# gwlucastrig/gridfour

Hardware: NVIDIA B200
Metric: GVRS tile decode GB/s of raw samples (config 3 shard, 180x240 tiles) (higher is better)
Workload: dtype int32

## Files before the change

### gridfour_b200/csrc/g4_lsop_fast.cu

```cuda
#include <cuda.h>
#include <cstdio>
#include <type_traits>
#include "g4_kernels.h"
#include "g4_predict.cuh"
#include "g4_lsop_common.cuh"

namespace g4 {

namespace {

constexpr int kTextThreads = 512;
constexpr int kTextThreadsSmall = 256;
constexpr uint32_t kTextSmallTile = 16384;
constexpr uint32_t kTextSubBits = 320;
constexpr int kExcWords = 128;
constexpr int kExcCap = (kExcWords - 2) / 2;
constexpr uint32_t kTextLookback = 96;
constexpr int kStageWordsPerThread = 22;
constexpr int kSpillWords = 8;
constexpr int kResidGuard = 256;
constexpr float kMagicHalf = 6291456.0f;
constexpr float kMagicHalfUp = 6291456.5f;
constexpr float kMagicInt = 12582912.0f;
constexpr float kRange = 2097152.0f;

__device__ __forceinline__ uint32_t smem_u32(const void* p) { return uint32_t(__cvta_generic_to_shared(p)); }
__host__ __device__ constexpr size_t text_fast_bytes(uint32_t stageWords) {
  return (offsetof(CanonFastShared, sw) + size_t(stageWords + 8u) * 4u + 127u) & ~size_t(127);
}
__device__ __forceinline__ void mbar_init(uint32_t bar, uint32_t count) {
  asm volatile("mbarrier.init.shared::cta.b64 [%0], %1;" ::"r"(bar), "r"(count));
}
__device__ __forceinline__ void mbar_expect_tx(uint32_t bar, uint32_t bytes) {
  asm volatile("mbarrier.arrive.expect_tx.shared::cta.b64 _, [%0], %1;" ::"r"(bar), "r"(bytes) : "memory");
}
__device__ __forceinline__ void mbar_wait(uint32_t bar, uint32_t parity) {
  uint32_t done = 0;
  while (!done)
    asm volatile("{ .reg .pred p; mbarrier.try_wait.parity.shared::cta.b64 p, [%1], %2; selp.u32 %0, 1, 0, p; }"
                 : "=r"(done)
                 : "r"(bar), "r"(parity)
                 : "memory");
}

__device__ __forceinline__ uint32_t image_offset(uint32_t w, int logW, uint32_t P, uint32_t k) {
  const uint32_t rr = k / w, pp = k - rr * w;
  return (rr + (pp >> logW)) * P + pp;
}

__device__ inline uint32_t warp_scan_inplace(int32_t* p, int n, uint32_t carry, int stride = 1) {
  const int lane = threadIdx.x & 31;
  for (int i0 = 0; i0 < n; i0 += 32) {
    const int i = i0 + lane;
    const uint32_t x = i < n ? uint32_t(p[i * stride]) : 0u;
    const uint32_t inc = warp_inclusive_scan(x);
    if (i < n) p[i * stride] = int32_t(carry + inc);
    carry += __shfl_sync(0xffffffffu, inc, 31);
  }
  __syncwarp();
  return carry;
}

__global__ void __launch_bounds__(kThreads, 3) lsop2_head_kernel(LsopFastArgs A, uint32_t maxPackBytes, int listBegin, int listEnd) {
  extern __shared__ __align__(16) unsigned char headSmem[];
  const DecodeArgs& a = A.a;
  const int lane = threadIdx.x & 31, warp = threadIdx.x >> 5;
  const int R = A.g.R, C = A.g.C;
  const uint32_t nInit = uint32_t(4 * R + 2 * C - 9);
  const size_t perWarp = ((sizeof(CanonWarpShared) + 15) & ~size_t(15)) + ((size_t(nInit) * 4 + 15) & ~size_t(15));
  CanonWarpShared& W = *reinterpret_cast<CanonWarpShared*>(headSmem + perWarp * warp);
  int32_t* init = reinterpret_cast<int32_t*>(headSmem + perWarp * warp + ((sizeof(CanonWarpShared) + 15) & ~size_t(15)));
  const int li = listBegin + blockIdx.x * kWarps + warp;
  if (li >= listEnd || li >= *a.listCount) return;
  const int tIdx = a.list[li];
  uint8_t* m = A.meta + size_t(tIdx) * kLsopMetaBytes;
  if (lane == 0) {
    *reinterpret_cast<uint32_t*>(m) = 0;
    A.exc[size_t(tIdx) * kExcWords] = 0;
  }
  const TileView t = tile_view(a.band, a.grid, tIdx);
  const uint8_t* packing = a.arena + a.offsets[tIdx];
  const uint32_t len = a.lens[tIdx];
  LsHeaderInfo h = parse_ls_header(packing, len, A.coef + size_t(tIdx) * 12, lane == 0);
  if (lane == 0 && a.lsopCks && h.ok && h.hasChecksum) { a.lsopCks[2 * tIdx] = 1u; a.lsopCks[2 * tIdx + 1] = h.valueChecksum; }
  if (!h.ok) {
    if (lane == 0) a.status[tIdx] = G4_ERR_FORMAT;
    return;
  }
  if (h.type != 2 || len + 96u > maxPackBytes) {
    if (lane == 0) A.defer[atomicAdd(A.deferCount, 1)] = tIdx;
    return;
  }
  BitSrc src;
  src.init(packing, len);
  canon_warp_parse_header(W, src, h.headerSize * 8u);
  int status = W.error ? G4_ERR_FORMAT : G4_OK;
  uint32_t endBit = 0;
  if (status == G4_OK) {
    uint32_t eb = 0, nv = 0;
    auto emit = [&](uint32_t k, int32_t v) { init[k] = v; };
    const bool ok = canon_warp_decode_text(W, src, W.textStart, nInit, emit, &eb, &nv) && nv == nInit;
    __syncwarp();
    if (lane == 0) {
      if (!ok) W.error = 1;
      W.textStart = eb;
    }
    __syncwarp();
    if (W.error) status = G4_ERR_FORMAT;
    endBit = W.textStart;
  }
  if (status == G4_OK) {
    canon_warp_parse_header(W, src, endBit);
    if (W.error) status = G4_ERR_FORMAT;
    else {
      for (int i = lane; i < kCanonSymbols; i += 32) {
        m[8 + i] = W.lens[i];
        reinterpret_cast<uint16_t*>(m + kLsopMetaSorted)[i] = W.sorted[i];
      }
      if (lane < 17) {
        reinterpret_cast<uint16_t*>(m + kLsopMetaFirst)[lane] = W.firstCode[lane];
        reinterpret_cast<uint16_t*>(m + kLsopMetaCount)[lane] = W.count[lane];
        reinterpret_cast<uint16_t*>(m + kLsopMetaOffset)[lane] = W.offset[lane];
      }
      if (lane == 0) *reinterpret_cast<uint32_t*>(m) = W.textStart;
    }
  }
  if (status == G4_OK) {
    int32_t* sA = init;
    int32_t* sB = sA + (C - 1);
    int32_t* sC = sB + (R - 1);
    int32_t* sD = sC + (C - 1);
    int32_t* sE = sD + (R - 2);
    const uint32_t seed = uint32_t(h.seed);
    warp_scan_inplace(sA, C - 1, seed);
    warp_scan_inplace(sB, R - 1, seed);
    warp_scan_inplace(sC, C - 1, uint32_t(sB[0]) - seed);
    for (int i = lane; i < C - 1; i += 32) sC[i] = int32_t(uint32_t(sC[i]) + uint32_t(sA[i]));
    __syncwarp();
    warp_scan_inplace(sD, R - 2, uint32_t(sC[0]) - uint32_t(sB[0]));
    warp_scan_inplace(sE, R - 2, uint32_t(sC[C - 3]) - uint32_t(sC[C - 4]), 2);
    warp_scan_inplace(sE + 1, R - 2, uint32_t(sC[C - 2]) - uint32_t(sC[C - 3]), 2);
    int32_t* row0 = t.row(0);
    int32_t* row1 = t.row(1);
    for (int c = lane; c < C; c += 32) {
      row0[c] = c ? sA[c - 1] : int32_t(seed);
      row1[c] = c ? sC[c - 1] : sB[0];
    }
    int4* side = A.side + size_t(tIdx) * R;
    for (int r = lane; r < R; r += 32) {
      int4 s;
      if (r == 0) s = make_int4(int32_t(seed), sA[0], 0, 0);
      else if (r == 1) s = make_int4(sB[0], sC[0], 0, 0);
      else s = make_int4(sB[r - 1], int32_t(uint32_t(sB[r - 1]) + uint32_t(sD[r - 2])), sE[2 * (r - 2)], sE[2 * (r - 2) + 1]);
      side[r] = s;
    }
  }
  if (lane == 0) a.status[tIdx] = status;
}

struct ByteTileSink {
  static constexpr bool kPacked = true;
  uint8_t* tile;
  uint32_t* exc;
  int w;
  int logW;
  uint32_t P, Wm1;
  uint32_t addr;
  uint32_t rowBase;
  int left;
  int kAddr;
  int head;
  int cnt;
  uint64_t q;
  int excK, excSlot;
  int32_t excV;

  __device__ __forceinline__ void init(uint8_t* img, uint32_t* e, const LsopFastGeom& geom) {
    tile = img;
    exc = e;
    logW = geom.logW;
    w = geom.C - 4;
    P = uint32_t(geom.P);
    Wm1 = uint32_t(geom.W - 1);
  }
  __device__ __forceinline__ void begin(uint32_t k0) {
    const int rr = int(k0) / w, pp = int(k0) - rr * w;
    rowBase = uint32_t(rr) * P;
    const uint32_t a0 = rowBase + (uint32_t(pp) >> logW) * P + uint32_t(pp);
    head = pp & 3;
    addr = a0 & ~3u;
    left = w - (pp & ~3);
    kAddr = int(k0) - head;
    cnt = head;
    q = 0;
    excK = -1;
    excSlot = 0;
    excV = 0;
  }
  __device__ __forceinline__ int cur_k() const { return kAddr + cnt; }
  __device__ __forceinline__ void store_word() {
    if (head) {
      for (int i = head; i < 4; i++) tile[addr + i] = uint8_t(q >> (8 * i));
      head = 0;
    } else *reinterpret_cast<uint32_t*>(tile + addr) = uint32_t(q);
    q >>= 32;
    cnt -= 4;
    kAddr += 4;
    step();
  }
  __device__ __forceinline__ void step() {
    addr += 4;
    left -= 4;
    if ((addr & Wm1) == 0u) {
      addr += P;
      if (left == 0) {
        rowBase += P;
        addr = rowBase;
        left = w;
      }
    } else if (__builtin_expect(left == 0, 0)) {
      rowBase += P;
      addr = rowBase;
      left = w;
    }
  }
  __device__ __forceinline__ void put_word(uint32_t dw, int lo, int hi) {
    if (lo == 0 && hi >= 4) *reinterpret_cast<uint32_t*>(tile + addr) = dw;
    else
      for (int b = lo; b < hi && b < 4; b++) tile[addr + b] = uint8_t(dw >> (8 * b));
    step();
  }
  __device__ __forceinline__ void push(uint32_t bytes, int n) {
    q |= uint64_t(bytes) << (8 * cnt);
    cnt += n;
    if (cnt >= 4) store_word();
  }
  __device__ __forceinline__ int add_exception(int k, int32_t v) {
    const uint32_t slot = atomicAdd(exc, 1u);
    if (slot < uint32_t(kExcCap)) {
      exc[2 + 2 * slot] = uint32_t(k);
      exc[3 + 2 * slot] = uint32_t(v);
    }
    excK = k;
    excV = v;
    excSlot = int(slot);
    return int(slot);
  }
  __device__ __forceinline__ void put_rare(int32_t v) {
    add_exception(cur_k(), v);
    push(0u, 1);
  }
  __device__ __forceinline__ void amend(int nb, uint32_t bits) {
    const int kp = cur_k() - 1;
    if (kp == excK) {
      excV = int32_t((uint32_t(excV) << nb) | bits);
      if (excSlot < kExcCap) exc[3 + 2 * excSlot] = uint32_t(excV);
      return;
    }
    uint32_t b;
    if (cnt > head) {
      const int sh = 8 * (cnt - 1);
      b = uint32_t(q >> sh) & 0xffu;
      q &= ~(0xffull << sh);
    } else {
      const uint32_t o = image_offset(uint32_t(w), logW, P, uint32_t(kp));
      b = tile[o];
      tile[o] = 0;
    }
    add_exception(kp, int32_t(((b - 128u) << nb) | bits));
  }
  __device__ __forceinline__ void end() {
    for (int i = head; i < cnt; i++) tile[addr + i] = uint8_t(q >> (8 * i));
  }
};

constexpr int kSubRare = 4;
constexpr int kSubOverflow = 8;

struct PosCursor {
  uint32_t lo, hi, next, pos;
  __device__ __forceinline__ void init(const uint32_t* sw, uint32_t p) {
    const uint32_t i = p >> 5;
    lo = sw[i];
    hi = sw[i + 1];
    next = i + 2;
    pos = p;
  }
  __device__ __forceinline__ uint32_t peek() const { return __funnelshift_r(lo, hi, pos); }
  __device__ __forceinline__ void skip(const uint32_t* sw, uint32_t n) {
    const uint32_t np = pos + n;
    if ((np ^ pos) & 32u) {
      lo = hi;
      hi = sw[next++];
    }
    pos = np;
  }
};

struct ByteAcc {
  uint32_t acc, qc8, w;
  __device__ __forceinline__ void init() { acc = 0; qc8 = 0; w = 0; }
  __device__ __forceinline__ void append(uint32_t m24, uint32_t n8, uint32_t* slot, uint32_t slotWords, uint32_t* spill) {
    const uint32_t out = __funnelshift_l(acc, m24, qc8);
    acc = __funnelshift_r(acc, m24, n8);
    qc8 += n8;
    if (qc8 >= 32u) {
      if (w < slotWords) slot[w] = out;
      else if (w - slotWords < uint32_t(kSpillWords)) spill[w - slotWords] = out;
      w++;
      qc8 -= 32u;
    }
  }
  __device__ __forceinline__ void finish(uint32_t* slot, uint32_t slotWords, uint32_t* spill) {
    if (qc8) {
      const uint32_t out = acc >> (32u - qc8);
      if (w < slotWords) slot[w] = out;
      else if (w - slotWords < uint32_t(kSpillWords)) spill[w - slotWords] = out;
      w++;
    }
  }
};

__device__ __forceinline__ void text_stage_sub(const CanonFastShared& S, uint32_t nBits, uint32_t start, uint32_t limit, uint32_t* slot,
                                               uint32_t slotWords, uint32_t* spill, uint32_t* endOut, uint32_t* cntOut, int* flagOut) {
  PosCursor cur;
  cur.init(S.sw, start);
  const int lastFull = int(limit) - kFastLutBits;
  uint32_t c = 0, end;
  int flag = 0;
  ByteAcc A;
  A.init();
  for (;;) {
    if (int(cur.pos) <= lastFull) {
      const uint32_t m = S.mlut[cur.peek() & ((1u << kFastLutBits) - 1u)];
      const uint32_t n = m >> 28;
      if (n) {
        cur.skip(S.sw, (m >> 24) & 15u);
        c += n;
        A.append(m & 0xffffffu, (m >> 25) & 0x18u, slot, slotWords, spill);
        continue;
      }
    }
    const uint32_t e = S.lut[cur.peek() & ((1u << kFastLutBits) - 1u)];
    uint32_t byte;
    if (e - 1u < 0x7fffu) {
      if (cur.pos >= limit) { end = cur.pos; break; }
      cur.skip(S.sw, e >> 9);
      byte = e & 0xffu;
    } else {
      const uint32_t p0 = cur.pos;
      uint32_t after;
      const int sym = canon_fast_rare_symbol(S, e, p0, nBits, &after);
      if (sym < 0) { flag = 2; end = p0; break; }
      if (sym == kSymEsc2 || sym == kSymEsc8) {
        after += sym == kSymEsc2 ? 2u : 8u;
        if (after > nBits) { flag = 2; end = p0; break; }
        flag |= kSubRare;
        cur.init(S.sw, after);
        continue;
      }
      if (p0 >= limit) { end = p0; break; }
      if (sym == kSymEot) { flag |= 1; end = after; break; }
      if (sym == kSymNull) { flag |= kSubRare; byte = 0u; }
      else byte = uint32_t(sym);
      cur.init(S.sw, after);
    }
    c++;
    A.append(byte, 8u, slot, slotWords, spill);
  }
  A.finish(slot, slotWords, spill);
  if (A.w > slotWords + uint32_t(kSpillWords)) flag |= kSubOverflow;
  *endOut = end;
  *cntOut = c;
  *flagOut = flag;
}

__device__ __forceinline__ bool text_write_sub(const CanonFastShared& S, uint32_t nBits, uint32_t start, uint32_t limit, uint32_t k0,
                                            ByteTileSink& sink) {
  BitCursor cur;
  cur.init(S, start, limit);
  sink.begin(k0);
  bool have = false, ok = true;
  for (;;) {
    if (cur.rem >= kFastLutBits) {
      const uint32_t m = S.mlut[cur.peek() & ((1u << kFastLutBits) - 1u)];
      const uint32_t n = m >> 28;
      if (n) {
        cur.skip(S, (m >> 24) & 15u);
        sink.push(m & 0xffffffu, int(n));
        have = true;
        continue;
      }
    }
    const uint32_t e = S.lut[cur.peek() & ((1u << kFastLutBits) - 1u)];
    if (e - 1u < 0x7fffu) {
      if (cur.rem <= 0) break;
      cur.skip(S, e >> 9);
      sink.push(e & 0xffu, 1);
      have = true;
      continue;
    }
    const uint32_t p0 = cur.pos(limit);
    uint32_t after;
    const int sym = canon_fast_rare_symbol(S, e, p0, nBits, &after);
    if (sym < 0) { ok = false; break; }
    if (sym == kSymEsc2 || sym == kSymEsc8) {
      const int nb = sym == kSymEsc2 ? 2 : 8;
      if (!have || after + nb > nBits) { ok = false; break; }
      SmemBitSrc src{S.sw, nBits};
      sink.amend(nb, src.bits(after, nb));
      after += nb;
    } else {
      if (p0 >= limit || sym == kSymEot) break;
      if (sym == kSymNull) sink.put_rare(INT32_MIN);
      else sink.push(uint32_t(sym), 1);
      have = true;
    }
    cur.init(S, after, limit);
  }
  sink.end();
  return ok;
// ... 219 lines not shown
    const int tIdx = a.list[li];
    const uint8_t* m = A.meta + size_t(tIdx) * kLsopMetaBytes;
    const uint32_t T0 = *reinterpret_cast<const uint32_t*>(m);
    if (T0 == 0) { __syncthreads(); continue; }
    const uint8_t* packing = a.arena + a.offsets[tIdx];
    const uint32_t len = a.lens[tIdx];
    const uint32_t delta = uint32_t(reinterpret_cast<uintptr_t>(packing) & 15u);
    const uint8_t* src16 = packing - delta;
    const uint32_t span = len + delta, nBulk = span & ~15u;
    if (tid == 0 && nBulk) {
      mbar_expect_tx(bar, nBulk);
      asm volatile("cp.async.bulk.shared::cluster.global.mbarrier::complete_tx::bytes [%0], [%1], %2, [%3];" ::"r"(smem_u32(F.sw)), "l"(src16),
                   "r"(nBulk), "r"(bar)
                   : "memory");
    }
    if (tid < 64) {
      const uint32_t i = nBulk + uint32_t(tid);
      reinterpret_cast<uint8_t*>(F.sw)[i] = i < span ? src16[i] : uint8_t(0);
    }
    for (int i = tid; i < kCanonSymbols; i += NT) F.sorted[i] = reinterpret_cast<const uint16_t*>(m + kLsopMetaSorted)[i];
    if (tid < 17) {
      F.firstCode[tid] = reinterpret_cast<const uint16_t*>(m + kLsopMetaFirst)[tid];
      F.count[tid] = reinterpret_cast<const uint16_t*>(m + kLsopMetaCount)[tid];
      F.offset[tid] = reinterpret_cast<const uint16_t*>(m + kLsopMetaOffset)[tid];
    }
    if (tid == 0) F.error = 0;
    __syncthreads();
    bool ok = true;
    canon_fast_build_lut<NT>(F);
    if (nBulk) mbar_wait(bar, parity);
    parity ^= nBulk ? 1u : 0u;
    __syncthreads();
    int rc = ok ? 0 : 1;
    if (ok) {
      const uint32_t nInterior = uint32_t(A.g.R - 2) * uint32_t(A.g.C - 4);
      ByteTileSink sink;
      sink.init(tileImg, A.exc + size_t(tIdx) * kExcWords, A.g);
      if (tid == 0) asm volatile("cp.async.bulk.wait_group.read 0;" ::: "memory");
      rc = lsop_text_decode<NT>(F, span * 8u, T0 + 8u * delta, nInterior, uint32_t(A.g.tileBytes), sink,
                                reinterpret_cast<uint32_t*>(A.textStage) + size_t(blockIdx.x) * (kFastMaxSub * kSpillWords));
      if (rc == 2) {
        uint32_t endBit = 0, nv = 0;
        rc = (canon_fast_decode_text<ByteTileSink, NT, kTextSubBits>(F, span * 8u, T0 + 8u * delta, nInterior, 0u, sink, &endBit, &nv) &&
              nv == nInterior) ? 0 : 1;
      }
      ok = rc == 0;
    }
    __syncthreads();
    if (tid == 0) {
      if (rc == 1) a.status[tIdx] = G4_ERR_FORMAT;
      else if (A.exc[size_t(tIdx) * kExcWords] > uint32_t(kExcCap)) {
        A.exc[size_t(tIdx) * kExcWords] = uint32_t(kExcCap) + 1u;
        A.defer[atomicAdd(A.deferCount, 1)] = tIdx;
      }
      else {
        asm volatile("fence.proxy.async.shared::cta;" ::: "memory");
        uint8_t* dst = A.resid + kResidGuard + size_t(tIdx) * size_t(A.g.tilePitch);
        asm volatile("cp.async.bulk.global.shared::cta.bulk_group [%0], [%1], %2;" ::"l"(dst), "r"(smem_u32(tileImg)), "r"(uint32_t(A.g.tileBytes))
                     : "memory");
        asm volatile("cp.async.bulk.commit_group;" ::: "memory");
      }
    }
  }
  if (tid == 0) asm volatile("cp.async.bulk.wait_group 0;" ::: "memory");
}

#ifndef G4_WAVE_CTAS
#define G4_WAVE_CTAS 2
#endif
#ifndef G4_WAVE_WARPS
#define G4_WAVE_WARPS 8
#endif
constexpr int kWaveWarps = G4_WAVE_WARPS;
constexpr int kWaveChunkBytes = 4096;

__device__ __noinline__ int32_t wave_exception(const uint32_t* exc, int n, int k) {
  for (int i = 0; i < n; i++)
    if (int(exc[2 + 2 * i]) == k) return int32_t(exc[3 + 2 * i]);
  return -128;
}

__device__ __forceinline__ int wave_rowbuf_floats(int C) { return (C + 4 + 3) & ~3; }

template <int W, bool WIDE>
__global__ void __launch_bounds__(32 * kWaveWarps, G4_WAVE_CTAS) lsop3_wave_kernel(LsopFastArgs A, int* tileCounter, int listBegin, int listEnd) {
  extern __shared__ __align__(128) unsigned char waveSmem[];
  constexpr int CR = 128 / W;
  constexpr int NW = W / 4;
  constexpr int E = W - 4;
  const DecodeArgs& a = A.a;
  const int lane = threadIdx.x & 31, warp = threadIdx.x >> 5;
  const LsopFastGeom& G = A.g;
  const int R = G.R, C = G.C, nS = G.nStrips, P = G.P;
  const int rbFloats = wave_rowbuf_floats(C);
  unsigned char* ring = waveSmem + size_t(warp) * (2 * kWaveChunkBytes);
  float* rowbuf = reinterpret_cast<float*>(waveSmem + size_t(kWaveWarps) * (2 * kWaveChunkBytes)) + size_t(warp) * (2 * rbFloats);
  uint64_t* bars = reinterpret_cast<uint64_t*>(waveSmem + size_t(kWaveWarps) * (2 * kWaveChunkBytes) + size_t(kWaveWarps) * (2 * rbFloats) * sizeof(float)) + 2 * warp;
  const uint32_t bar0 = smem_u32(bars), ring0 = smem_u32(ring);
  const bool active = lane < nS, isFirst = lane == 0, isLast = lane == nS - 1;
  if (lane == 0) {
    mbar_init(bar0, 1);
    mbar_init(bar0 + 8, 1);
    asm volatile("fence.mbarrier_init.release.cluster;");
  }
  __syncwarp();
  uint32_t gchunk = 0;
  for (;;) {
  int li = 0;
  if (lane == 0) li = listBegin + atomicAdd(tileCounter, 1);
  li = __shfl_sync(0xffffffffu, li, 0);
  if (li >= listEnd || li >= *a.listCount) break;
  const int tIdx = a.list[li];
  if (a.status[tIdx] != G4_OK) continue;
  if (*reinterpret_cast<const uint32_t*>(A.meta + size_t(tIdx) * kLsopMetaBytes) == 0u) continue;
  const uint32_t* exc = A.exc + size_t(tIdx) * kExcWords;
  const int nExc = int(exc[0]);
  if (nExc > kExcCap) continue;
  const TileView t = tile_view(a.band, a.grid, tIdx);
  const uint8_t* img = A.resid + kResidGuard + size_t(tIdx) * size_t(G.tilePitch);
  const uint32_t chunkBytes = uint32_t(CR * P);
  const int nChunks = G.nChunks;
  auto issue = [&](int chunk) {
    const uint32_t g = gchunk + uint32_t(chunk);
    const uint32_t bar = bar0 + 8u * (g & 1u), dst = ring0 + uint32_t(kWaveChunkBytes) * (g & 1u);
    mbar_expect_tx(bar, chunkBytes);
    asm volatile("cp.async.bulk.shared::cluster.global.mbarrier::complete_tx::bytes [%0], [%1], %2, [%3];" ::"r"(dst),
                 "l"(img + size_t(chunk) * chunkBytes), "r"(chunkBytes), "r"(bar)
                 : "memory");
  };
  if (lane == 0) issue(0);

  float u[12];
#pragma unroll
  for (int i = 0; i < 12; i++) u[i] = active ? A.coef[size_t(tIdx) * 12 + i] : 0.f;
  for (int c = lane; c < rbFloats; c += 32) {
    rowbuf[c] = c < C ? float(t.row(0)[c]) : 0.f;
    rowbuf[rbFloats + c] = c < C ? float(t.row(1)[c]) : 0.f;
  }
  const int4* side = A.side + size_t(tIdx) * R;
  const bool needSide = active && (isFirst || isLast);
  uint32_t rr = active ? uint32_t(-lane) : 0x40000000u;
  const uint32_t nRowsIn = uint32_t(R - 2);
  int4 sideCur = make_int4(0, 0, 0, 0), sideNext = make_int4(0, 0, 0, 0);
  if (needSide && rr < nRowsIn) sideNext = side[2 + rr];
  const int4* sideAt = side + 3 - lane;
  char* rowp = reinterpret_cast<char*>(t.base + int64_t(2 - lane) * t.pitch + lane * W);
  const int64_t rowStep = int64_t(t.pitch) * 4;
  const uint32_t ringLane = ring0 + uint32_t(lane * W);
  uint32_t ringAt = ringLane;
  const uint32_t rb0 = smem_u32(rowbuf) + uint32_t(lane * W) * 4u, rb1 = rb0 + uint32_t(rbFloats) * 4u;
  const int wInterior = C - 4;
  uint32_t badBits = 0;
  float a0[W + 4], a1[W + 4], a2[W + 4];
#pragma unroll
  for (int i = 0; i < W + 4; i++) { a0[i] = 0.f; a1[i] = 0.f; a2[i] = 0.f; }
  int32_t pa = 0, pb = 0;
  float h0 = 0.f, h1 = 0.f;
  __syncwarp();

  auto step = [&](float (&am2)[W + 4], float (&am1)[W + 4], float (&cur)[W + 4], const int s) {
    if ((s & (CR - 1)) == 0) {
      const int chunk = s / CR;
      if (chunk < nChunks) {
        if (lane == 0 && chunk + 1 < nChunks) issue(chunk + 1);
        const uint32_t g = gchunk + uint32_t(chunk);
        mbar_wait(bar0 + 8u * (g & 1u), (g >> 1) & 1u);
      }
      ringAt = ringLane + uint32_t(kWaveChunkBytes) * ((gchunk + uint32_t(chunk)) & 1u);
    }
    const bool valid = rr < nRowsIn;
    const bool first = rr == 0u;
    if (s < nS) {
     if (first) {
#pragma unroll
      for (int i = 0; i < W + 4; i += 4) {
        float4 x, y;
        asm volatile("ld.shared.v4.f32 {%0, %1, %2, %3}, [%4];" : "=f"(x.x), "=f"(x.y), "=f"(x.z), "=f"(x.w) : "r"(rb0 + 4u * i));
        asm volatile("ld.shared.v4.f32 {%0, %1, %2, %3}, [%4];" : "=f"(y.x), "=f"(y.y), "=f"(y.z), "=f"(y.w) : "r"(rb1 + 4u * i));
        am2[i] = x.x; am2[i + 1] = x.y; am2[i + 2] = x.z; am2[i + 3] = x.w;
        am1[i] = y.x; am1[i + 1] = y.y; am1[i + 2] = y.z; am1[i + 3] = y.w;
      }
      h0 = am1[W + 2];
      h1 = am1[W + 3];
     }
    }
    sideCur = sideNext;
    if (needSide && rr + 1u < nRowsIn) sideNext = *sideAt;
    sideAt++;
    uint32_t rw[NW];
    {
      const uint32_t at = ringAt;
      ringAt += uint32_t(P);
      if constexpr (NW == 1) asm volatile("ld.shared.b32 %0, [%1];" : "=r"(rw[0]) : "r"(at));
      else if constexpr (NW == 2) asm volatile("ld.shared.v2.b32 {%0, %1}, [%2];" : "=r"(rw[0]), "=r"(rw[1]) : "r"(at));
      else asm volatile("ld.shared.v4.b32 {%0, %1, %2, %3}, [%4];" : "=r"(rw[0]), "=r"(rw[1]), "=r"(rw[2]), "=r"(rw[3]) : "r"(at));
    }
    float l2 = __shfl_up_sync(0xffffffffu, am1[W], 1), l1 = __shfl_up_sync(0xffffffffu, am1[W + 1], 1);
    int32_t li2 = __shfl_up_sync(0xffffffffu, pa, 1), li1 = __shfl_up_sync(0xffffffffu, pb, 1);
    if (isFirst) { li2 = sideCur.x; li1 = sideCur.y; l2 = float(li2); l1 = float(li1); }
    cur[0] = l2;
    cur[1] = l1;
    bool general = false;
    if (nExc > 0) {
      bool z = false;
#pragma unroll
      for (int i = 0; i < NW; i++) z = z || ((rw[i] - 0x01010101u) & ~rw[i] & 0x80808080u) != 0u;
      general = __any_sync(0xffffffffu, z && valid);
    }
    int32_t oi[W];
    uint32_t accLo = 0, accHi = 0;
    auto cells = [&](auto genTag) {
      constexpr bool GEN = decltype(genTag)::value;
#pragma unroll
      for (int j = 0; j < W; j++) {
        constexpr int dummy = 0;
        (void)dummy;
        const int c = j + 2;
        if (j == 2) {
          const float s0 = __shfl_down_sync(0xffffffffu, cur[2], 1), s1 = __shfl_down_sync(0xffffffffu, cur[3], 1);
          am1[W + 2] = first ? h0 : s0;
          am1[W + 3] = first ? h1 : s1;
        }
        float p = u[0] * cur[c - 1];
        p = p + u[1] * am1[c - 1];
        p = p + u[2] * am1[c];
        p = p + u[3] * am1[c + 1];
        p = p + u[4] * am1[c + 2];
        p = p + u[5] * cur[c - 2];
        p = p + u[6] * am1[c - 2];
        p = p + u[7] * am2[c - 2];
        p = p + u[8] * am2[c - 1];
        p = p + u[9] * am2[c];
        p = p + u[10] * am2[c + 1];
        p = p + u[11] * am2[c + 2];
        const float t1 = __fadd_rd(p, kMagicHalf);
        if (j < E) accLo |= __float_as_uint(t1) ^ 0x4A800000u;
        else accHi |= __float_as_uint(t1) ^ 0x4A800000u;
        const float t2 = __fadd_rd(t1, kMagicHalfUp);
        const uint32_t word = rw[j >> 2];
        const float xj = __uint_as_float(__byte_perm(word, 0x4B400000u, 0x7640 + (j & 3)));
        float fv = t2 + (xj - (2.f * kMagicInt + 128.f));
        int32_t iv;
        if constexpr (GEN) {
          const uint32_t byte = (word >> (8 * (j & 3))) & 0xffu;
          int32_t ex = int32_t(byte) - 128;
          if (byte == 0u && valid) ex = wave_exception(exc, nExc, int(rr) * wInterior + lane * W + j);
          iv = int32_t(uint32_t(__float_as_int(t2)) - 0x4B400000u + uint32_t(ex));
          fv = float(iv);
        } else iv = int32_t(uint32_t(__float_as_int(t2)) + __float_as_uint(xj) - 0x96800080u);
        if (j == E || j == E + 1) {
          const int32_t prev = j == 0 ? li1 : oi[j > 0 ? j - 1 : 0];
          const int32_t sv = int32_t(uint32_t(prev) + uint32_t(j == E ? sideCur.z : sideCur.w));
          if (isLast) { iv = sv; fv = float(sv); }
        }
        oi[j] = iv;
        cur[c] = fv;
      }
    };
    if (general) cells(std::true_type{});
    else cells(std::false_type{});
    if (valid) badBits |= (accLo | (isLast ? 0u : accHi)) & 0xFF800000u;
    if (valid) {
      if constexpr (W == 4) *reinterpret_cast<int4*>(rowp) = make_int4(li2, li1, oi[0], oi[1]);
      else {
        if (WIDE) {
          asm volatile("st.global.v8.b32 [%0], {%1,%2,%3,%4,%5,%6,%7,%8};" ::"l"(rowp), "r"(li2), "r"(li1), "r"(oi[0]), "r"(oi[1]), "r"(oi[2]),
                       "r"(oi[3]), "r"(oi[4]), "r"(oi[5])
                       : "memory");
          if constexpr (W == 16)
            asm volatile("st.global.v8.b32 [%0], {%1,%2,%3,%4,%5,%6,%7,%8};" ::"l"(rowp + 32), "r"(oi[6]), "r"(oi[7]), "r"(oi[8]), "r"(oi[9]),
                         "r"(oi[10]), "r"(oi[11]), "r"(oi[12]), "r"(oi[13])
                         : "memory");
        } else {
          *reinterpret_cast<int4*>(rowp) = make_int4(li2, li1, oi[0], oi[1]);
          *reinterpret_cast<int4*>(rowp + 16) = make_int4(oi[2], oi[3], oi[4], oi[5]);
          if constexpr (W == 16) {
            *reinterpret_cast<int4*>(rowp + 32) = make_int4(oi[6], oi[7], oi[8], oi[9]);
            *reinterpret_cast<int4*>(rowp + 48) = make_int4(oi[10], oi[11], oi[12], oi[13]);
          }
        }
      }
    }
    pa = oi[W - 2];
    pb = oi[W - 1];
    rr++;
    rowp += rowStep;
    __syncwarp();
  };

  const int nSteps = G.nSteps;
#pragma unroll 1
  for (int s = 0; s < nSteps; s += 3) {
    step(a0, a1, a2, s);
    step(a1, a2, a0, s + 1);
    step(a2, a0, a1, s + 2);
  }
  if (__any_sync(0xffffffffu, badBits != 0u)) {
    if (lane == 0) A.defer[atomicAdd(A.deferCount, 1)] = tIdx;
  }
  gchunk += uint32_t(nChunks);
  }
}

size_t head_smem_bytes(const LsopFastGeom& g) {
  const size_t nInit = size_t(4 * g.R + 2 * g.C - 9);
  return size_t(kWarps) * (((sizeof(CanonWarpShared) + 15) & ~size_t(15)) + ((nInit * 4 + 15) & ~size_t(15))) + 16;
}
uint32_t text_stage_words(const LsopFastGeom& g) {
  uint32_t w = uint32_t((uint64_t(g.R) * uint64_t(g.C) * 5 / 8 + 3) / 4) + 128u;
  if (w < 512u) w = 512u;
  return (w + 255u) & ~255u;
}
size_t text_smem_bytes(const LsopFastGeom& g) { return text_fast_bytes(text_stage_words(g)) + size_t(g.tileBytes); }
bool text_small(const LsopFastGeom& g) { return uint32_t(g.R) * uint32_t(g.C) <= kTextSmallTile; }
size_t wave_smem_bytes(const LsopFastGeom& g) {
  const size_t rbFloats = size_t((g.C + 4 + 3) & ~3);
  return size_t(kWaveWarps) * (2 * kWaveChunkBytes) + size_t(kWaveWarps) * (2 * rbFloats) * sizeof(float) + size_t(kWaveWarps) * 16;
}

template <int W>
cudaError_t launch_wave(const LsopFastArgs& A, int nCtas, int nTilesUpper, int* tileCounter, cudaStream_t s) {
  const size_t smem = wave_smem_bytes(A.g);
  cudaError_t e;
  if (A.g.wide) {
    if ((e = cudaFuncSetAttribute(lsop3_wave_kernel<W, true>, cudaFuncAttributeMaxDynamicSharedMemorySize, int(smem))) != cudaSuccess) return e;
    lsop3_wave_kernel<W, true><<<nCtas, 32 * kWaveWarps, smem, s>>>(A, tileCounter, 0, nTilesUpper);
  } else {
    if ((e = cudaFuncSetAttribute(lsop3_wave_kernel<W, false>, cudaFuncAttributeMaxDynamicSharedMemorySize, int(smem))) != cudaSuccess) return e;
    lsop3_wave_kernel<W, false><<<nCtas, 32 * kWaveWarps, smem, s>>>(A, tileCounter, 0, nTilesUpper);
  }
  return cudaGetLastError();
}

}

bool lsop_fast_geometry(const g4_band_desc& band, const void* grid, LsopFastGeom* out) {
  LsopFastGeom g{};
  g.R = band.tile_rows;
  g.C = band.tile_cols;
  if (g.R < 6 || g.C < 16 || (g.C & 3) != 0 || (band.grid_pitch & 3) != 0 || (reinterpret_cast<uintptr_t>(grid) & 15) != 0) return false;
  if (g.C <= 128) g.W = 4;
  else if (g.C <= 256 && (g.C & 7) == 0) g.W = 8;
  else if (g.C <= 512 && (g.C & 15) == 0) g.W = 16;
  else return false;
  g.logW = g.W == 4 ? 2 : g.W == 8 ? 3 : 4;
  g.nStrips = (g.C - 2 + g.W - 1) / g.W;
  g.P = g.nStrips * g.W;
  g.nSteps = g.R - 2 + g.nStrips - 1;
  g.chunkRows = 128 / g.W;
  g.nChunks = (g.nSteps + g.chunkRows - 1) / g.chunkRows;
  g.tileBytes = g.nChunks * g.chunkRows * g.P;
  g.tilePitch = g.tileBytes;
  g.wide = ((band.grid_pitch & 7) == 0 && (reinterpret_cast<uintptr_t>(grid) & 31) == 0) ? 1 : 0;
  if (text_smem_bytes(g) > 224u * 1024u || head_smem_bytes(g) > 224u * 1024u || wave_smem_bytes(g) > 224u * 1024u) return false;
  *out = g;
  return true;
}
size_t lsop_fast_side_bytes(const LsopFastGeom& g, int nTiles) { return size_t(nTiles) * size_t(g.R) * sizeof(int4); }
size_t lsop_fast_exc_bytes(int nTiles) { return size_t(nTiles) * kExcWords * sizeof(uint32_t); }
size_t lsop_fast_stage_bytes(int smCount) { return size_t(smCount) * 4 * kFastMaxSub * kSpillWords * sizeof(uint32_t); }
size_t lsop_fast_resid_bytes(const LsopFastGeom& g, int nTiles) { return size_t(kResidGuard) + size_t(nTiles) * size_t(g.tilePitch) + 4096; }

cudaError_t launch_lsop_decode_fast(const LsopFastArgs& A, int nTilesUpper, int smCount, int* textCounter, cudaStream_t s, int* launches) {
  const LsopFastGeom& g = A.g;
  {
    cudaError_t e = cudaFuncSetAttribute(lsop2_head_kernel, cudaFuncAttributeMaxDynamicSharedMemorySize, int(head_smem_bytes(g)));
    if (e == cudaSuccess)
      e = text_small(g) ? cudaFuncSetAttribute(lsop2_text_kernel<kTextThreadsSmall>, cudaFuncAttributeMaxDynamicSharedMemorySize, int(text_smem_bytes(g)))
                        : cudaFuncSetAttribute(lsop2_text_kernel<kTextThreads>, cudaFuncAttributeMaxDynamicSharedMemorySize, int(text_smem_bytes(g)));
    if (e != cudaSuccess) return e;
  }
  const uint32_t stageWords = text_stage_words(g);
  const int nCtasWarp = (nTilesUpper + kWarps - 1) / kWarps;
  lsop2_head_kernel<<<nCtasWarp, kThreads, head_smem_bytes(g), s>>>(A, stageWords * 4u, 0, nTilesUpper);
  cudaError_t e = cudaGetLastError();
  if (e != cudaSuccess) return e;
  LsopFastArgs T = A;
  T.a.counter = textCounter;
  const size_t textSmem = text_smem_bytes(g);
  int perSm = int((227u * 1024u) / (textSmem + 1024));
  const int perSmCap = text_small(g) ? 4 : 2;
  if (perSm < 1) perSm = 1;
  if (perSm > perSmCap) perSm = perSmCap;
  int ctas = smCount * perSm;
  if (ctas > nTilesUpper) ctas = nTilesUpper;
  if (text_small(g)) lsop2_text_kernel<kTextThreadsSmall><<<ctas, kTextThreadsSmall, textSmem, s>>>(T, stageWords, 0, nTilesUpper);
  else lsop2_text_kernel<kTextThreads><<<ctas, kTextThreads, textSmem, s>>>(T, stageWords, 0, nTilesUpper);
  if ((e = cudaGetLastError()) != cudaSuccess) return e;
  int nCtasWave = (nTilesUpper + kWaveWarps - 1) / kWaveWarps;
  if (nCtasWave > smCount * G4_WAVE_CTAS) nCtasWave = smCount * G4_WAVE_CTAS;
  int* waveCounter = textCounter + 1;
  e = g.W == 4 ? launch_wave<4>(A, nCtasWave, nTilesUpper, waveCounter, s) : g.W == 8 ? launch_wave<8>(A, nCtasWave, nTilesUpper, waveCounter, s)
                                                                                          : launch_wave<16>(A, nCtasWave, nTilesUpper, waveCounter, s);
  if (e != cudaSuccess) return e;
  if (launches) *launches += 3;
  return cudaSuccess;
}

}
```

Baseline: 876.7.

## Rewrite LSOP head kernel with static smem, global init buffer, and parallel text decode

```diff
diff --git a/gridfour_b200/csrc/g4_lsop_fast.cu b/gridfour_b200/csrc/g4_lsop_fast.cu
--- a/gridfour_b200/csrc/g4_lsop_fast.cu
+++ b/gridfour_b200/csrc/g4_lsop_fast.cu
@@ -61,18 +61,272 @@
   return carry;
 }
 
-__global__ void __launch_bounds__(kThreads, 3) lsop2_head_kernel(LsopFastArgs A, uint32_t maxPackBytes, int listBegin, int listEnd) {
-  extern __shared__ __align__(16) unsigned char headSmem[];
+constexpr int kHeadLutBits = 9;
+static_assert(offsetof(CanonWarpShared, ctLut) == offsetof(CanonWarpShared, lut8) + sizeof(CanonWarpShared::lut8) &&
+                  sizeof(CanonWarpShared::lut8) + sizeof(CanonWarpShared::ctLut) >= (2u << kHeadLutBits),
+              "the head kernel's text LUT spans lut8 and ctLut");
+__device__ __forceinline__ uint16_t* head_lut(CanonWarpShared& W) {
+  return reinterpret_cast<uint16_t*>(reinterpret_cast<unsigned char*>(&W) + offsetof(CanonWarpShared, lut8));
+}
+__device__ __forceinline__ const uint16_t* head_lut(const CanonWarpShared& W) {
+  return reinterpret_cast<const uint16_t*>(reinterpret_cast<const unsigned char*>(&W) + offsetof(CanonWarpShared, lut8));
+}
+
+__device__ inline void head_parse_table(CanonWarpShared& W, const BitSrc& src, uint32_t startBit, bool textLut) {
+  const int lane = threadIdx.x & 31;
+  __syncwarp();
+  if (lane == 0) {
+    W.error = 0;
+    uint32_t pos = startBit + 1;
+    int k = 0, prior = 0;
+    while (k < 20 && !W.error) {
+      if (pos + 5 > src.nBits) { W.error = 1; break; }
+      int index = int(src.bits(pos, 5));
+      pos += 5;
+      int n = 1, val = index;
+      if (index <= 15) prior = index;
+      else if (index == 16) { n = int(src.bits(pos, 2)) + 3; pos += 2; val = prior; }
+      else if (index == 17) { n = int(src.bits(pos, 3)) + 3; pos += 3; val = 0; prior = 0; }
+      else if (index == 18) { n = int(src.bits(pos, 7)) + 11; pos += 7; val = 0; prior = 0; }
+      else continue;
+      if (k + n > 20) { W.error = 1; break; }
+      for (int i = 0; i < n; i++) W.lens[k++] = uint8_t(val);
+    }
+    if (!W.error && !canon_build_tables(W.lens, 20, W.ctFirst, W.ctCount, W.ctOffset, W.ctSorted)) W.error = 1;
+    W.textStart = pos;
+  }
+  __syncwarp();
+  if (W.error) return;
+  for (int e = lane; e < 256; e += 32) {
+    uint32_t v = __brev(uint32_t(e));
+    uint16_t entry = 0;
+    for (int len = 1; len <= 8; len++) {
+      uint32_t d = (v >> (32 - len)) - W.ctFirst[len];
+      if (d < W.ctCount[len]) { entry = uint16_t(W.ctSorted[W.ctOffset[len] + d] | (len << 8)); break; }
+    }
+    W.ctLut[e] = entry;
+  }
+  for (int i = lane; i < (kCanonSymbols + 4) / 4; i += 32) reinterpret_cast<uint32_t*>(W.lens)[i] = 0u;
+  __syncwarp();
+  if (lane == 0) {
+    GlobalCursor cur;
+    cur.init(src, W.textStart);
+    int prior = 0;
+    for (int i = 0; i < kCanonSymbols;) {
+      if (cur.pos >= src.nBits) { W.error = 1; break; }
+      int test;
+      uint32_t e = W.ctLut[cur.peek() & 0xffu];
+      if (e) { test = int(e & 0xffu); cur.skip(e >> 8); }
+      else {
+        uint32_t p = cur.pos;
+        test = canon_slow_symbol(W.ctFirst, W.ctCount, W.ctOffset, W.ctSorted, src, &p, 9);
+        if (test >= 0) cur.init(src, p);
+      }
+      if (test < 0) { W.error = 1; break; }
+      int n = 1, val = 0;
+      if (test <= 15) { val = test; prior = test; }
+      else if (test == 16) { n = int(cur.peek() & 3u) + 3; cur.skip(2); val = prior; }
+      else if (test == 17) { n = int(cur.peek() & 7u) + 3; cur.skip(3); prior = 0; }
+      else if (test == 18) { n = int(cur.peek() & 127u) + 11; cur.skip(7); prior = 0; }
+      if (i + n > kCanonSymbols) { W.error = 1; break; }
+      W.lens[i] = uint8_t(0x80 | val);
+      i += n;
+    }
+    W.textStart = cur.pos;
+  }
+  if (lane < 17) W.cnt32[lane] = 0;
+  __syncwarp();
+  if (W.error) return;
+  {
+    uint32_t carry = 0;
+    for (int i0 = 0; i0 < kCanonSymbols; i0 += 32) {
+      const int i = i0 + lane;
+      uint32_t x = i < kCanonSymbols ? W.lens[i] : 0u;
+#pragma unroll
+      for (int d = 1; d < 32; d <<= 1) {
+        const uint32_t y = __shfl_up_sync(0xffffffffu, x, d);
+        if (lane >= d && x == 0u) x = y;
+      }
+      if (x == 0u) x = carry;
+      carry = __shfl_sync(0xffffffffu, x, 31);
+      const int l = int(x & 15u);
+      if (i < kCanonSymbols) {
+        W.lens[i] = uint8_t(l);
+        if (l) atomicAdd(&W.cnt32[l], 1u);
+      }
+    }
+  }
+  __syncwarp();
+  if (lane == 0) {
+    if (W.lens[kSymEot] == 0) W.error = 1;
+    uint32_t code = 0, off = 0;
+    W.count[0] = 0; W.firstCode[0] = 0; W.offset[0] = 0; W.next[0] = 0;
+    W.count[16] = 0; W.firstCode[16] = 0; W.offset[16] = 0; W.next[16] = 0;
+    for (int l = 1; l <= 15; l++) {
+      uint32_t c = W.cnt32[l];
+      W.firstCode[l] = uint16_t(code);
+      W.offset[l] = uint16_t(off);
+      W.count[l] = uint16_t(c);
+      W.next[l] = off;
+      if (code + c > (1u << l)) W.error = 1;
+      code = (code + c) << 1;
+      off += c;
+    }
+  }
+  __syncwarp();
+  if (W.error) return;
+  for (int i0 = 0; i0 < kCanonSymbols; i0 += 32) {
+    const int i = i0 + lane;
+    const int l = i < kCanonSymbols ? W.lens[i] : 0;
+    const uint32_t same = __match_any_sync(0xffffffffu, l);
+    if (l) {
+      const uint32_t rank = __popc(same & ((1u << lane) - 1u));
+      W.sorted[W.next[l] + rank] = uint16_t(i);
+    }
+    __syncwarp();
+    if (l && (same & ((1u << lane) - 1u)) == 0) W.next[l] += __popc(same);
+    __syncwarp();
+  }
+  if (!textLut) return;
+  for (int e = lane; e < (1 << kHeadLutBits); e += 32) {
+    uint32_t v = __brev(uint32_t(e));
+    uint16_t entry = 0;
+    for (int len = 1; len <= kHeadLutBits; len++) {
+      uint32_t d = (v >> (32 - len)) - W.firstCode[len];
+      if (d < W.count[len]) {
+        uint32_t sym = W.sorted[W.offset[len] + d];
+        entry = uint16_t(sym | (uint32_t(len) << 9) | (sym >= 256 ? kFastSpecial : 0u));
+        break;
+      }
+    }
+    head_lut(W)[e] = entry;
+  }
+  __syncwarp();
+}
+
+__device__ __forceinline__ int head_symbol(const CanonWarpShared& W, const BitSrc& src, GlobalCursor& cur) {
+  const uint32_t e = head_lut(W)[cur.peek() & ((1u << kHeadLutBits) - 1u)];
+  if (e) {
+    cur.skip((e >> 9) & 15u);
+    return int(e & 0x1ffu);
+  }
+  uint32_t p = cur.pos;
+  const int sym = canon_slow_symbol(W.firstCode, W.count, W.offset, W.sorted, src, &p, kHeadLutBits + 1);
+  if (sym >= 0) cur.init(src, p);
+  return sym;
+}
+
+__device__ inline void head_count(const CanonWarpShared& W, const BitSrc& src, uint32_t start, uint32_t limit, uint32_t* endOut,
+                                  uint32_t* cntOut, int* flagOut) {
+  GlobalCursor cur;
+  cur.init(src, start);
+  uint32_t c = 0, end;
+  int flag = 0;
+  for (;;) {
+    const uint32_t p0 = cur.pos;
+    const int sym = head_symbol(W, src, cur);
+    if (sym < 0) { flag = 2; end = p0; break; }
+    if (sym == kSymEsc2 || sym == kSymEsc8) {
+      cur.skip(sym == kSymEsc2 ? 2u : 8u);
+      if (cur.pos > src.nBits) { flag = 2; end = p0; break; }
+      continue;
+    }
+    if (p0 >= limit) { end = p0; break; }
+    if (sym == kSymEot) { flag = 1; end = cur.pos; break; }
+    c++;
+  }
+  *endOut = end;
+  *cntOut = c;
+  *flagOut = flag;
+}
+
+__device__ inline bool head_decode_text(const CanonWarpShared& W, const BitSrc& src, uint32_t T0, uint32_t nInit, int32_t* init,
+                                        uint32_t* endBit) {
+  const int lane = threadIdx.x & 31;
+  uint32_t kBase = 0, regionStart = T0;
+  for (;;) {
+    if (regionStart >= src.nBits) return false;
+    uint32_t regionEnd = regionStart + 32u * kWarpSubBits;
+    if (regionEnd > src.nBits) regionEnd = src.nBits;
+    const uint32_t lo = regionStart + uint32_t(lane) * kWarpSubBits;
+    const bool has = lo < regionEnd;
+    uint32_t limit = lo + kWarpSubBits;
+    if (limit > regionEnd) limit = regionEnd;
+    uint32_t start = lane == 0 ? regionStart : 0xffffffffu, end = regionEnd, cnt = 0;
+    int flag = 0;
+    if (has) {
+      uint32_t from = lo;
+      if (lane > 0 && limit - lo > 48u) from = limit - 48u;
+      head_count(W, src, from, limit, &end, &cnt, &flag);
+    }
+    for (int pass = 0; pass < 34; pass++) {
+      uint32_t ns = __shfl_up_sync(0xffffffffu, end, 1);
+      if (lane == 0) ns = regionStart;
+      const bool ch = has && ns != start;
+      if (ch) {
+        start = ns;
+        head_count(W, src, start, limit, &end, &cnt, &flag);
+      }
+      if (__ballot_sync(0xffffffffu, ch) == 0) break;
+    }
+    const uint32_t flagged = __ballot_sync(0xffffffffu, has && flag != 0);
+    const int fe = flagged ? __ffs(flagged) - 1 : 32;
+    if (fe < 32 && __shfl_sync(0xffffffffu, flag, fe) == 2) return false;
+    const bool mine = has && lane <= fe;
+    const uint32_t c = mine ? cnt : 0u;
+    const uint32_t inc = warp_inclusive_scan(c);
+    const uint32_t total = __shfl_sync(0xffffffffu, inc, 31);
+    if (kBase + total > nInit) return false;
+    bool bad = false;
+    if (mine) {
+      uint32_t k = kBase + inc - c;
+      GlobalCursor cur;
+      cur.init(src, start);
+      bool have = false;
+      uint32_t v = 0;
+      for (;;) {
+        const uint32_t p0 = cur.pos;
+        const int sym = head_symbol(W, src, cur);
+        if (sym < 0) { bad = true; break; }
+        if (sym == kSymEsc2 || sym == kSymEsc8) {
+          if (!have) { bad = true; break; }
+          const uint32_t nb = sym == kSymEsc2 ? 2u : 8u;
+          v = (v << nb) | (cur.peek() & ((1u << nb) - 1u));
+          cur.skip(nb);
+          continue;
+        }
+        if (p0 >= limit || sym == kSymEot) break;
+        if (have) init[k++] = int32_t(v);
+        have = true;
+        v = sym == kSymNull ? uint32_t(INT32_MIN) : uint32_t(sym - 128);
+      }
+      if (have) init[k] = int32_t(v);
+    }
+    if (__ballot_sync(0xffffffffu, bad)) return false;
+    kBase += total;
+    if (fe < 32) {
+      *endBit = __shfl_sync(0xffffffffu, end, fe);
+      return kBase == nInit;
+    }
+    const uint32_t hasMask = __ballot_sync(0xffffffffu, has);
+    regionStart = __shfl_sync(0xffffffffu, end, 31 - __clz(hasMask));
+  }
+}
+
+#ifndef G4_HEAD_CTAS
+#define G4_HEAD_CTAS 6
+#endif
+__global__ void __launch_bounds__(kThreads, G4_HEAD_CTAS) lsop2_head_kernel(LsopFastArgs A, uint32_t maxPackBytes, int listBegin, int listEnd) {
+  __shared__ CanonWarpShared WS[kWarps];
   const DecodeArgs& a = A.a;
   const int lane = threadIdx.x & 31, warp = threadIdx.x >> 5;
   const int R = A.g.R, C = A.g.C;
   const uint32_t nInit = uint32_t(4 * R + 2 * C - 9);
-  const size_t perWarp = ((sizeof(CanonWarpShared) + 15) & ~size_t(15)) + ((size_t(nInit) * 4 + 15) & ~size_t(15));
-  CanonWarpShared& W = *reinterpret_cast<CanonWarpShared*>(headSmem + perWarp * warp);
-  int32_t* init = reinterpret_cast<int32_t*>(headSmem + perWarp * warp + ((sizeof(CanonWarpShared) + 15) & ~size_t(15)));
+  CanonWarpShared& W = WS[warp];
   const int li = listBegin + blockIdx.x * kWarps + warp;
   if (li >= listEnd || li >= *a.listCount) return;
   const int tIdx = a.list[li];
+  int32_t* init = reinterpret_cast<int32_t*>(A.resid + kResidGuard + size_t(tIdx) * size_t(A.g.tilePitch));
   uint8_t* m = A.meta + size_t(tIdx) * kLsopMetaBytes;
   if (lane == 0) {
     *reinterpret_cast<uint32_t*>(m) = 0;
@@ -81,7 +335,11 @@
   const TileView t = tile_view(a.band, a.grid, tIdx);
   const uint8_t* packing = a.arena + a.offsets[tIdx];
   const uint32_t len = a.lens[tIdx];
-  LsHeaderInfo h = parse_ls_header(packing, len, A.coef + size_t(tIdx) * 12, lane == 0);
+  LsHeaderInfo h = parse_ls_header(packing, len, nullptr, false);
+  if (len >= 3u + 4u + 48u && lane < 12) {
+    const uint32_t at = (packing[1] & 0x40) == 0 ? 1u : 2u;
+    if (packing[at] == 12) A.coef[size_t(tIdx) * 12 + lane] = __uint_as_float(load_le32(packing + at + 5u + 4u * uint32_t(lane)));
+  }
   if (lane == 0 && a.lsopCks && h.ok && h.hasChecksum) { a.lsopCks[2 * tIdx] = 1u; a.lsopCks[2 * tIdx + 1] = h.valueChecksum; }
   if (!h.ok) {
     if (lane == 0) a.status[tIdx] = G4_ERR_FORMAT;
@@ -93,30 +351,19 @@
   }
   BitSrc src;
   src.init(packing, len);
-  canon_warp_parse_header(W, src, h.headerSize * 8u);
+  head_parse_table(W, src, h.headerSize * 8u, true);
   int status = W.error ? G4_ERR_FORMAT : G4_OK;
   uint32_t endBit = 0;
   if (status == G4_OK) {
-    uint32_t eb = 0, nv = 0;
-    auto emit = [&](uint32_t k, int32_t v) { init[k] = v; };
-    const bool ok = canon_warp_decode_text(W, src, W.textStart, nInit, emit, &eb, &nv) && nv == nInit;
+    const bool ok = head_decode_text(W, src, W.textStart, nInit, init, &endBit);
     __syncwarp();
-    if (lane == 0) {
-      if (!ok) W.error = 1;
-      W.textStart = eb;
-    }
-    __syncwarp();
-    if (W.error) status = G4_ERR_FORMAT;
-    endBit = W.textStart;
+    if (!ok) status = G4_ERR_FORMAT;
   }
   if (status == G4_OK) {
-    canon_warp_parse_header(W, src, endBit);
+    head_parse_table(W, src, endBit, false);
     if (W.error) status = G4_ERR_FORMAT;
     else {
-      for (int i = lane; i < kCanonSymbols; i += 32) {
-        m[8 + i] = W.lens[i];
-        reinterpret_cast<uint16_t*>(m + kLsopMetaSorted)[i] = W.sorted[i];
-      }
+      for (int i = lane; i < kCanonSymbols; i += 32) reinterpret_cast<uint16_t*>(m + kLsopMetaSorted)[i] = W.sorted[i];
       if (lane < 17) {
         reinterpret_cast<uint16_t*>(m + kLsopMetaFirst)[lane] = W.firstCode[lane];
         reinterpret_cast<uint16_t*>(m + kLsopMetaCount)[lane] = W.count[lane];
@@ -942,10 +1189,6 @@
   }
 }
 
-size_t head_smem_bytes(const LsopFastGeom& g) {
-  const size_t nInit = size_t(4 * g.R + 2 * g.C - 9);
-  return size_t(kWarps) * (((sizeof(CanonWarpShared) + 15) & ~size_t(15)) + ((nInit * 4 + 15) & ~size_t(15))) + 16;
-}
 uint32_t text_stage_words(const LsopFastGeom& g) {
   uint32_t w = uint32_t((uint64_t(g.R) * uint64_t(g.C) * 5 / 8 + 3) / 4) + 128u;
   if (w < 512u) w = 512u;
@@ -992,7 +1235,8 @@
   g.tileBytes = g.nChunks * g.chunkRows * g.P;
   g.tilePitch = g.tileBytes;
   g.wide = ((band.grid_pitch & 7) == 0 && (reinterpret_cast<uintptr_t>(grid) & 31) == 0) ? 1 : 0;
-  if (text_smem_bytes(g) > 224u * 1024u || head_smem_bytes(g) > 224u * 1024u || wave_smem_bytes(g) > 224u * 1024u) return false;
+  if (text_smem_bytes(g) > 224u * 1024u || wave_smem_bytes(g) > 224u * 1024u) return false;
+  if (size_t(4 * g.R + 2 * g.C - 9) * 4u > size_t(g.tilePitch)) return false;
   *out = g;
   return true;
 }
@@ -1004,15 +1248,13 @@
 cudaError_t launch_lsop_decode_fast(const LsopFastArgs& A, int nTilesUpper, int smCount, int* textCounter, cudaStream_t s, int* launches) {
   const LsopFastGeom& g = A.g;
   {
-    cudaError_t e = cudaFuncSetAttribute(lsop2_head_kernel, cudaFuncAttributeMaxDynamicSharedMemorySize, int(head_smem_bytes(g)));
-    if (e == cudaSuccess)
-      e = text_small(g) ? cudaFuncSetAttribute(lsop2_text_kernel<kTextThreadsSmall>, cudaFuncAttributeMaxDynamicSharedMemorySize, int(text_smem_bytes(g)))
+    cudaError_t e = text_small(g) ? cudaFuncSetAttribute(lsop2_text_kernel<kTextThreadsSmall>, cudaFuncAttributeMaxDynamicSharedMemorySize, int(text_smem_bytes(g)))
                         : cudaFuncSetAttribute(lsop2_text_kernel<kTextThreads>, cudaFuncAttributeMaxDynamicSharedMemorySize, int(text_smem_bytes(g)));
     if (e != cudaSuccess) return e;
   }
   const uint32_t stageWords = text_stage_words(g);
   const int nCtasWarp = (nTilesUpper + kWarps - 1) / kWarps;
-  lsop2_head_kernel<<<nCtasWarp, kThreads, head_smem_bytes(g), s>>>(A, stageWords * 4u, 0, nTilesUpper);
+  lsop2_head_kernel<<<nCtasWarp, kThreads, 0, s>>>(A, stageWords * 4u, 0, nTilesUpper);
   cudaError_t e = cudaGetLastError();
   if (e != cudaSuccess) return e;
   LsopFastArgs T = A;
diff --git a/probes/profile_lsop_head.py b/probes/profile_lsop_head.py
--- /dev/null
+++ b/probes/profile_lsop_head.py
@@ -0,0 +1,85 @@
+import argparse
+import json
+import os
+import subprocess
+import sys
+
+ROOT = os.path.dirname(os.path.dirname(os.path.abspath(__file__)))
+sys.path.insert(0, ROOT)
+sys.dont_write_bytecode = True
+
+KERNELS = {"H": "lsop2_head_kernel", "T": "lsop2_text_kernel", "W": "lsop3_wave_kernel"}
+
+
+def gpu_info(index):
+    q = subprocess.run(["nvidia-smi", "-i", str(index), "--query-gpu=name,power.limit,clocks.max.sm", "--format=csv,noheader"],
+                       capture_output=True, text=True, timeout=30)
+    name, power, clock = [x.strip() for x in q.stdout.strip().split(",")]
+    return {"name": name, "power_limit": power, "max_sm_clock": clock}
+
+
+def main():
+    ap = argparse.ArgumentParser()
+    ap.add_argument("--steps", type=int, default=20)
+    ap.add_argument("--out", default=None, help="also write the JSON result to this file")
+    args = ap.parse_args()
+
+    import torch
+    from torch.profiler import ProfilerActivity, profile
+
+    import gridfour_b200 as g4
+
+    dev = torch.device("cuda", 0)
+    torch.cuda.set_device(dev)
+    info = gpu_info(0)
+    stream = torch.cuda.Stream(dev)
+    torch.cuda.set_stream(stream)
+    ctx = g4.Context(0, stream.cuda_stream)
+    spec = g4.CodecSpecification(default=False)
+    spec.addCompressionCodec("GvrsHuffman", g4.CodecHuffman)
+    spec.addCompressionCodec("GvrsDeflate", g4.CodecDeflate)
+    spec.addCompressionCodec("LSOP12", g4.LsEncoder12, g4.LsDecoder12)
+    master = g4.CodecMaster(spec, ctx)
+
+    tr, tc, rows, cols = 180, 240, 5400, 86400
+    z = torch.empty((rows, cols), dtype=torch.int32, device=dev)
+    ctx.fill_terrain(z.data_ptr(), 0, 0, 0, rows, cols)
+    batch = master.encodeTiles(z, tr, tc)
+    out = torch.empty_like(z)
+    master.decodeTiles(batch, out=out)
+    torch.cuda.synchronize(dev)
+    assert torch.equal(out, z)
+    n = int(batch.lens.numel())
+
+    with profile(activities=[ProfilerActivity.CUDA]) as prof:
+        for _ in range(args.steps):
+            master.decodeTiles(batch, out=out)
+        torch.cuda.synchronize(dev)
+    total_us, per = 0.0, {k: {"us": 0.0, "calls": 0} for k in KERNELS}
+    for e in prof.events():
+        if e.device_type != torch.autograd.DeviceType.CUDA:
+            continue
+        us = e.device_time if hasattr(e, "device_time") else e.cuda_time
+        total_us += us
+        for k, sub in KERNELS.items():
+            if sub in e.name:
+                per[k]["us"] += us
+                per[k]["calls"] += 1
+    result = {
+        "what": "LSOP12 fast-path kernel times per decode of the config-3 shard (%d tiles of %dx%d int32, codecs "
+                "GvrsHuffman+GvrsDeflate+LSOP12), torch.profiler device times, mean over %d decodes" % (n, tr, tc, args.steps),
+        "gpu": info, "steps": args.steps, "n_tiles": n,
+        "ms_per_decode": {KERNELS[k]: per[k]["us"] / 1e3 / args.steps for k in KERNELS},
+        "launches_per_decode": {KERNELS[k]: per[k]["calls"] / args.steps for k in KERNELS},
+        "ms_per_decode_all_device_activity": total_us / 1e3 / args.steps,
+    }
+    line = json.dumps(result)
+    print(line)
+    if args.out:
+        os.makedirs(os.path.dirname(os.path.abspath(args.out)), exist_ok=True)
+        with open(args.out, "w") as f:
+            f.write(json.dumps(result, indent=1) + "\n")
+
+
+if __name__ == "__main__":
+    main()
```

Result: no change. 883.6, median of 6 (+0.8%).
